# YunjiKim/Unsupervised-Keypoint-Learning-for-Guiding-Class-conditional-Video-Prediction

Measured on AMD Instinct MI355X. Metric: detector_translator train frames/sec @128x128 K=15, higher is better.
Workload: dtype f32

## Files before the change

include/kpx.h:

```cpp
#ifndef KPX_H
#define KPX_H

#include <stddef.h>
#include <stdint.h>

#ifdef __cplusplus
extern "C" {
#endif

#define KPX_EINVAL (-1)
#define KPX_ABI_VERSION 25

enum { KPX_ACT_NONE = 0, KPX_ACT_RELU = 1, KPX_ACT_LRELU = 2 , KPX_ACT_TANH = 3  };

int kpx_abi_version(void);

int kpx_reload_env(void);

enum { KPX_ARITH_F32 = 0, KPX_ARITH_BF16 = 1 };

size_t kpx_conv2d_fwd_workspace_bytes(int N, int Ho, int Wo, int Cin, int Cout, int KH, int KW);
int kpx_conv2d_fwd_f32(const float* x, int N, int Hi, int Wi, int Cin, int ldx,
                       const float* w_hwio, int KH, int KW, const float* bias,
                       float* y, int Ho, int Wo, int Cout, int ldy,
// ... 65 lines not shown
                         float* moving_mean, float* moving_var, float decay, float* y, int ldy, int act, void* scratch, void* stream);
int kpx_bn_train_bwd_f32(const float* dy, int lddy, const float* x, int ldx, size_t P, int groups, int C,
                         const float* mean, const float* invstd, const float* gamma, const float* beta, int act,
                         float* dx, int lddx, float* dgamma, float* dbeta, int accumulate,
                         const float* tile_stats, size_t tiles_per_group, void* scratch, void* stream);
int kpx_bn_train_fwd_bf16(const void* x, size_t P, int groups, int C, int ldx, const float* tile_stats, size_t tiles_per_group,
                          float eps, const float* gamma, const float* beta, float* mean, float* invstd,
                          float* moving_mean, float* moving_var, float decay, void* y, int ldy, int y_f32, int act, void* scratch, void* stream);
int kpx_bn_train_bwd_bf16(const void* dy, int lddy, int dy_f32, const void* x, int ldx, size_t P, int groups, int C,
                          const float* mean, const float* invstd, const float* gamma, const float* beta, int act,
                          void* dx, int lddx, float* dgamma, float* dbeta, int accumulate,
                          const float* tile_stats, size_t tiles_per_group, void* scratch, void* stream);
int kpx_bn_invstd_f32(const float* var, int C, float eps, float* invstd, void* stream);
int kpx_bn_apply_f32(const float* x, size_t P, int C, int ldx, const float* mean, const float* invstd,
                     const float* gamma, const float* beta, float* y, int ldy, int act, void* stream);
int kpx_bn_fold_conv_f32(const float* w, const float* bias, size_t rows, int C, const float* gamma, const float* beta,
                         const float* moving_mean, const float* moving_var, float eps, float* w_out, float* b_out, void* stream);

int kpx_conv3x3_wino43_eligible(int N, int H, int W, int K, int Nn, int ldin, const void* in_ptr);
size_t kpx_wino43_u_bytes(int Cin, int Cout);
int kpx_wino43_filter_transform_f32(const float* w_hwio, int Cin, int Cout, int dgrad, float* u, void* stream);
int kpx_wino43_filter_transform_batch_f32(const void* descs_dev, int n, void* stream);
int kpx_conv3x3_wino43_f32(const float* in, int N, int H, int W, int K, int ldin, const float* u, const float* bias,
                           float* out, int Nn, int ldout, int act, const float* mask_y, int ld_mask, float* pool_y, int ld_pool,
                           float* tile_stats, const float* bn_y, int ld_bn_y, const float* bn_beta, void* stream);
size_t kpx_conv3x3_wino43_stats_tiles(int N, int H, int W);
int kpx_conv3x3_wino43b_eligible(int N, int H, int W, int K, int Nn, int ldin, const void* in_ptr);
size_t kpx_wino43b_u_bytes(int Cin, int Cout);
int kpx_wino43b_filter_transform_f32(const float* w_hwio, int Cin, int Cout, int dgrad, void* u, void* stream);
int kpx_wino43b_filter_transform_batch_f32(const void* descs_dev, int n, void* stream);
int kpx_conv3x3_wino43b_f32(const float* in, int N, int H, int W, int K, int ldin, const void* u, const float* bias,
                            float* out, int Nn, int ldout, int act, const float* mask_y, int ld_mask, float* pool_y, int ld_pool,
                            float* tile_stats, const float* bn_y, int ld_bn_y, const float* bn_beta, void* stream);
int kpx_conv3x3_c16_eligible(int N, int H, int W, int K, int Nn, int ldin, int ldout, const void* in_ptr);
int kpx_conv3x3_c16_f32(const float* in, int N, int H, int W, int K, int ldin, const float* w_hwio, int dgrad, const float* bias,
                        float* out, int ldout, int act, float* tile_stats, void* stream);
int kpx_resize2x_fwd_f32(const float* x, int N, int H, int W, int C, int ldx, float* y, int ldy, void* stream);
int kpx_resize2x_bwd_f32(const float* dy, int N, int H, int W, int C, int lddy, float* dx, int lddx, void* stream);

int kpx_copy_channels_f32(const float* src, int ldsrc, float* dst, int lddst, size_t P, int C, void* stream);

size_t kpx_keypoint_head_scratch_bytes(int B, int H, int W, int K);
int kpx_keypoint_head_fwd_f32(const float* logits, int B, int H, int W, int K,
                              float* mu, float* prob_y, float* prob_x, void* scratch, void* stream);
int kpx_keypoint_head_bwd_f32(const float* dmu, const float* mu, const float* prob_y, const float* prob_x,
                              int B, int H, int W, int K, float* dlogits, void* stream);

size_t kpx_keypoint_head_proj_scratch_bytes(int B, int H, int W, int C, int K);
int kpx_keypoint_head_proj_eligible(int B, int H, int W, int C, int K);
int kpx_keypoint_head_proj_fwd_f32(const float* x, const float* wk, const float* bias, int B, int H, int W, int C, int K,
                                   float* mu, float* prob_y, float* prob_x, float* xs_y, float* xs_x, void* scratch, void* stream);
int kpx_keypoint_head_proj_bwd_f32(const float* dmu, const float* mu, const float* prob_y, const float* prob_x,
                                   const float* xs_y, const float* xs_x, const float* wk, int B, int H, int W, int C, int K,
                                   float* dx, float* dw, float* db, int accumulate, void* scratch, void* stream);

int kpx_gaussian_maps_fwd_f32(const float* mu, int B, int K, int H, int W, double inv_std, float* maps, int ldy, void* stream);
int kpx_gaussian_maps_bwd_f32(const float* dmaps, int lddy, const float* mu, int B, int K, int H, int W, double inv_std,
                              float* dmu, void* stream);

int kpx_point_maps_rgb_f32(const float* mu, int N, int K, int H, int W, double inv_std, const float* colors, float* out, void* stream);

int kpx_point_seq_strip_rgb_f32(const float* mu, int N, int T, int K, int H, int W, double inv_std, const float* colors, int recolour,
                                float* out, void* stream);

#define KPX_SUMMARY_SLICES 64
enum { KPX_PREMAP_IDENTITY = 0, KPX_PREMAP_X255 = 1, KPX_PREMAP_UNIT255 = 2, KPX_PREMAP_UNIT255_CLIP = 3 };
// ... 264 lines not shown
```

unsupervised-keypoint-learning-for-guiding-class-conditional-video-prediction_amd/_lib.py:

```python
import ctypes
import os
from ctypes import c_double, c_float, c_int, c_size_t, c_void_p

import torch

_HERE = os.path.dirname(os.path.abspath(__file__))
LIB_PATH = os.environ.get('KPX_LIB') or os.path.join(_HERE, 'libkpx_hip.so')


class KpxError(RuntimeError):
    pass


if not os.path.exists(LIB_PATH):
    raise ImportError(
        'libkpx_hip.so not found at %s -- build it first: python -c "import __graft_entry__ as g; g.build()" '
        '(or `make -C %s/csrc`). There is no CPU / PyTorch fallback for the hot path.' % (LIB_PATH, _HERE))

lib = ctypes.CDLL(LIB_PATH)

P = c_void_p
ABI_VERSION = 25
SIGNATURES = {
    'kpx_abi_version': (c_int, []),
    'kpx_reload_env': (c_int, []),
    'kpx_conv2d_fwd_workspace_bytes': (c_size_t, [c_int, c_int, c_int, c_int, c_int, c_int, c_int]),
    'kpx_conv2d_fwd_f32': (c_int, [P, c_int, c_int, c_int, c_int, c_int, P, c_int, c_int, P,
                                   P, c_int, c_int, c_int, c_int, c_int, c_int, c_int, c_int, c_int, P, c_size_t, P]),
    'kpx_conv2d_dgrad_workspace_bytes': (c_size_t, [c_int, c_int, c_int, c_int, c_int, c_int, c_int, c_int]),
    'kpx_conv2d_dgrad_f32': (c_int, [P, c_int, c_int, c_int, c_int, c_int, P, c_int, c_int,
                                     P, c_int, c_int, c_int, c_int, c_int, c_int, c_int, c_int, P, c_size_t, P]),
    'kpx_conv2d_dgrad_act_f32': (c_int, [P, c_int, c_int, c_int, c_int, c_int, P, c_int, c_int,
                                         P, c_int, c_int, c_int, c_int, c_int, c_int, c_int, c_int, P, c_int, c_int, P, c_size_t, P]),
    'kpx_conv2d_wgrad_workspace_bytes': (c_size_t, [c_int, c_int, c_int, c_int, c_int, c_int, c_int]),
    'kpx_conv2d_wgrad_f32': (c_int, [P, c_int, c_int, c_int, c_int, c_int, P, c_int, c_int, c_int, c_int,
                                     P, c_int, c_int, c_int, c_int, c_int, c_int, P, c_size_t, P]),
    'kpx_conv2d_wgrad_plan': (c_int, [P, c_int, c_int, c_int, c_int, c_int, P, c_int, c_int, c_int, c_int,
                                      c_int, c_int, c_int, c_int, c_int, c_int, P, P, P]),
    'kpx_wino_u_bytes': (c_size_t, [c_int, c_int]),
    'kpx_wino_filter_transform_f32': (c_int, [P, c_int, c_int, c_int, P, P]),
    'kpx_wino_filter_transform_batch_f32': (c_int, [P, c_int, P]),
    'kpx_conv3x3_wino_eligible': (c_int, [c_int, c_int, c_int, c_int, c_int, c_int, P]),
    'kpx_conv3x3_wino_f32': (c_int, [P, c_int, c_int, c_int, c_int, c_int, P, P, P, c_int, c_int, c_int, P, P, c_int, P, P]),
    'kpx_conv3x3_c16_eligible': (c_int, [c_int, c_int, c_int, c_int, c_int, c_int, c_int, P]),
    'kpx_conv3x3_c16_f32': (c_int, [P, c_int, c_int, c_int, c_int, c_int, P, c_int, P, P, c_int, c_int, P, P]),
    'kpx_conv3x3_wino43_eligible': (c_int, [c_int, c_int, c_int, c_int, c_int, c_int, P]),
    'kpx_wino43_u_bytes': (c_size_t, [c_int, c_int]),
    'kpx_wino43_filter_transform_f32': (c_int, [P, c_int, c_int, c_int, P, P]),
    'kpx_wino43_filter_transform_batch_f32': (c_int, [P, c_int, P]),
    'kpx_conv3x3_wino43_f32': (c_int, [P, c_int, c_int, c_int, c_int, c_int, P, P, P, c_int, c_int, c_int, P, c_int, P, c_int, P, P, c_int, P, P]),
    'kpx_conv3x3_wino43b_eligible': (c_int, [c_int, c_int, c_int, c_int, c_int, c_int, P]),
    'kpx_wino43b_u_bytes': (c_size_t, [c_int, c_int]),
    'kpx_wino43b_filter_transform_f32': (c_int, [P, c_int, c_int, c_int, P, P]),
    'kpx_wino43b_filter_transform_batch_f32': (c_int, [P, c_int, P]),
    'kpx_conv3x3_wino43b_f32': (c_int, [P, c_int, c_int, c_int, c_int, c_int, P, P, P, c_int, c_int, c_int, P, c_int, P, c_int, P, P, c_int, P, P]),
    'kpx_conv3x3_wino43_stats_tiles': (c_size_t, [c_int, c_int, c_int]),
    'kpx_conv3x3_wino_stats_tiles': (c_size_t, [c_int, c_int, c_int]),
    'kpx_conv3x3_bf16s_weights_bytes': (c_size_t, [c_int, c_int]),
    'kpx_conv3x3_bf16s_eligible': (c_int, [c_int, c_int, c_int, c_int, c_int, c_int, P]),
    'kpx_conv3x3_bf16s_stats_tiles': (c_int, [c_int, c_int, c_int, c_int, c_int]),
    'kpx_conv3x3_bf16s_prepare_f32': (c_int, [P, c_int, c_int, c_int, P, P]),
    'kpx_conv3x3_bf16s_prepare_batch_f32': (c_int, [P, c_int, P]),
    'kpx_conv3x3_bf16s': (c_int, [P, c_int, c_int, c_int, c_int, c_int, P, P, P, c_int, c_int, c_int, c_int, P, c_int, P, P]),
    'kpx_conv2d_fwd_bf16': (c_int, [P, c_int, c_int, c_int, c_int, c_int, P, c_int, c_int, P, P, c_int, c_int, c_int, c_int, c_int, c_int, c_int, c_int, c_int, P, c_size_t, P]),
    'kpx_conv2d_dgrad_bf16': (c_int, [P, c_int, c_int, c_int, c_int, c_int, P, c_int, c_int, P, c_int, c_int, c_int, c_int, c_int, c_int, c_int, c_int, P, c_int, c_int, P, c_size_t, P]),
    'kpx_conv2d_wgrad_bf16': (c_int, [P, c_int, c_int, c_int, c_int, c_int, P, c_int, c_int, c_int, c_int, P, c_int, c_int, c_int, c_int, c_int, P, c_size_t, P]),
    'kpx_conv_image_fwd_bf16': (c_int, [P, c_int, c_int, c_int, c_int, P, c_int, c_int, P, P, c_int, c_int, c_int, c_int, c_int, c_int, c_int, c_int, P]),
    'kpx_conv_image_dgrad_bf16': (c_int, [P, c_int, c_int, c_int, c_int, c_int, P, c_int, c_int, P, c_int, c_int, c_int, c_int, c_int, c_int, c_int, P]),
    'kpx_conv_image_wgrad_bf16': (c_int, [P, c_int, c_int, c_int, c_int, c_int, P, c_int, c_int, c_int, c_int, P, c_int, c_int, c_int, c_int, c_int, P, c_size_t, P]),
    'kpx_conv3x3_wgrad_bf16_eligible': (c_int, [c_int, c_int, c_int, c_int, c_int, c_int, c_int, P, P]),
    'kpx_conv3x3_wgrad_bf16_workspace_bytes': (c_size_t, [c_int, c_int, c_int, c_int, c_int]),
    'kpx_conv3x3_wgrad_bf16': (c_int, [P, c_int, c_int, c_int, c_int, c_int, P, c_int, c_int, P, P, c_size_t, P]),
    'kpx_conv3x3_bf16s_bnbwd': (c_int, [P, c_int, c_int, c_int, c_int, c_int, P, P, c_int, c_int, P, c_int, P, P, P]),
    'kpx_cast_channels': (c_int, [P, c_int, P, c_int, c_size_t, c_int, c_int, P]),
    'kpx_chan_sum_bf16': (c_int, [P, c_size_t, c_int, c_int, P, P, P]),
    'kpx_bn_train_fwd_bf16': (c_int, [P, c_size_t, c_int, c_int, c_int, P, c_size_t, c_float, P, P, P, P, P, P, c_float, P, c_int, c_int, c_int, P, P]),
    'kpx_bn_train_bwd_bf16': (c_int, [P, c_int, c_int, P, c_int, c_size_t, c_int, c_int, P, P, P, P, c_int, P, c_int, P, P, c_int, P, c_size_t, P, P]),
    'kpx_act_bwd_bf16': (c_int, [P, P, P, c_size_t, c_int, P]),
    'kpx_resize2x_fwd_bf16': (c_int, [P, c_int, c_int, c_int, c_int, c_int, P, c_int, P]),
    'kpx_resize2x_bwd_bf16': (c_int, [P, c_int, c_int, c_int, c_int, c_int, P, c_int, P]),
    'kpx_maxpool2_fwd_bf16': (c_int, [P, c_int, c_int, c_int, c_int, P, P]),
    'kpx_vgg_feat_bwd_bf16': (c_int, [P, c_size_t, P, c_float, P, c_int, c_int, c_int, c_int, P, P]),
    'kpx_l1_pair_fwd_bf16': (c_int, [P, c_size_t, P, P, P]),
    'kpx_act_bwd_f32': (c_int, [P, P, P, c_size_t, c_int, P]),
    'kpx_chan_reduce_scratch_bytes': (c_size_t, [c_int]),
    'kpx_chan_sum_f32': (c_int, [P, c_size_t, c_int, c_int, P, P, P]),
    'kpx_bn_invstd_f32': (c_int, [P, c_int, c_float, P, P]),
    'kpx_bn_fold_conv_f32': (c_int, [P, P, c_size_t, c_int, P, P, P, P, c_float, P, P, P]),
# ... 111 lines not shown
```

unsupervised-keypoint-learning-for-guiding-class-conditional-video-prediction_amd/csrc/conv_wino43b.hip:

```cpp
#include "kpx_bf16.h"
#include "kpx_env.h"
#include "wino43_options.h"
#include <type_traits>

#define W4B_ROWSLOTS 146
#define W4B_ROWSLOTS_PACK 154
#define W4B_NPIECES 44
#define W4B_RAW_BYTES (W4B_NPIECES * 1024)
#define W4B_ACC_OFF (2 * W4B_RAW_BYTES)
#define W4B_NLDS 4
#ifndef W4B_DMA_IN_T
#define W4B_DMA_IN_T 1
#endif
#ifndef W4B_U_AUX
#define W4B_U_AUX 0
#endif
#ifndef W4B_RING
#define W4B_RING 6
#endif
#if W4B_RING == 6
#define W4B_RING3 18
#else
#define W4B_RING3 27
#endif
#define W4B_STR2(x) #x
#define W4B_STR(x) W4B_STR2(x)
#define W4B_EPI_BYTES (36 * 32 * 32 * 4)
#define W4B_MAIN_BYTES (W4B_ACC_OFF + 4 * W4B_NLDS * 4096)

struct Wino43bGeom {
    const float* x; float* y; const void* U; const float* bias;
    int N, H, W, Cin, ldx, Cout, ldy, act;
    int Kp, Np;
    int tiles_y, tiles_x;
    const float* mask_y; int ld_mask;
    float* pool_y; int ld_pool;
    float* stats;
    const float* bn_beta;
};

__device__ __forceinline__ void w4b_split8(const float* __restrict__ v, u32x4* __restrict__ f) {
#if defined(W4B_EXP) && (W4B_EXP & 1)
#pragma unroll
    for (int m = 0; m < 4; ++m) { f[0][m] = kpx_bits(v[2 * m]); f[1][m] = kpx_bits(v[2 * m + 1]); f[2][m] = kpx_bits(v[m]); }
    return;
#endif
#pragma unroll
    for (int m = 0; m < 4; ++m) {
        unsigned p[3];
        kpx_split2<3>(v[2 * m], v[2 * m + 1], p);
        f[0][m] = p[0]; f[1][m] = p[1]; f[2][m] = p[2];
    }
}

struct KpxWino43bDesc { const float* w; unsigned* u; int cin, cout, dgrad, reserved; };

__constant__ double w4b_G[6][3] = {{0.25, 0.0, 0.0}, {-1.0 / 6.0, -1.0 / 6.0, -1.0 / 6.0}, {-1.0 / 6.0, 1.0 / 6.0, -1.0 / 6.0},
                                   {1.0 / 24.0, 1.0 / 12.0, 1.0 / 6.0}, {1.0 / 24.0, -1.0 / 12.0, 1.0 / 6.0}, {0.0, 0.0, 1.0}};

__device__ __forceinline__ void w4b_transform_filter(const float* __restrict__ w, int Cin, int Cout, bool dg, size_t idx, int Kp, int Np, unsigned* __restrict__ Ub) {
    const int K = dg ? Cout : Cin, Nn = dg ? Cin : Cout;
    const int KS = Kp >> 4, NB = Np >> 5, C8 = Kp >> 3;
    const int n = (int)(idx % (size_t)Np);
    const int c8 = (int)((idx / (size_t)Np) % (size_t)C8), i = (int)(idx / ((size_t)Np * C8));
    const double gi0 = w4b_G[i][0], gi1 = w4b_G[i][1], gi2 = w4b_G[i][2];
    float u[6][8];
    float g[9][8];
    const bool vec = dg && 8 * c8 + 8 <= K && n < Nn && (Cout & 3) == 0 && ((reinterpret_cast<uintptr_t>(w) & 15) == 0);
    if (vec) {
#pragma unroll
        for (int tp = 0; tp < 9; ++tp) {
            const f32x4* src = reinterpret_cast<const f32x4*>(w + ((size_t)(8 - tp) * Cin + n) * Cout + 8 * c8);
            const f32x4 a = src[0], b = src[1];
#pragma unroll
            for (int e = 0; e < 4; ++e) { g[tp][e] = a[e]; g[tp][4 + e] = b[e]; }
        }
    } else {
#pragma unroll
        for (int tp = 0; tp < 9; ++tp)
#pragma unroll
            for (int e = 0; e < 8; ++e) {
                const int c = 8 * c8 + e;
                g[tp][e] = !(c < K && n < Nn) ? 0.f : dg ? w[((size_t)(8 - tp) * Cin + n) * Cout + c] : w[((size_t)tp * Cin + c) * Cout + n];
            }
    }
// ... 606 lines not shown
```

unsupervised-keypoint-learning-for-guiding-class-conditional-video-prediction_amd/csrc/kpx_bf16.h:

```cpp
#pragma once
#include "kpx_common.h"

typedef __bf16 bf16x8 __attribute__((ext_vector_type(8)));
typedef unsigned int u32x4 __attribute__((ext_vector_type(4)));
typedef unsigned int u32x2 __attribute__((ext_vector_type(2)));
typedef __attribute__((address_space(3))) void* lds_ptr_t;

#define KPX_BUF_OOB 0x7ffffff0

template <int V> struct kpx_ic { static constexpr int value = V; };

static inline bool kpx_aligned16(const void* a, const void* b = nullptr, const void* c = nullptr) {
    return ((((uintptr_t)a) | ((uintptr_t)b) | ((uintptr_t)c)) & 15) == 0;
}

__device__ __forceinline__ unsigned kpx_bits(float v) { return __builtin_bit_cast(unsigned, v); }
__device__ __forceinline__ float kpx_float(unsigned v) { return __builtin_bit_cast(float, v); }
__device__ __forceinline__ unsigned kpx_pack_hi(unsigned a, unsigned b) { return __builtin_amdgcn_perm(b, a, 0x07060302u); }
__device__ __forceinline__ unsigned kpx_pack2(float a, float b) {
    typedef __bf16 bf16x2 __attribute__((ext_vector_type(2)));
    const bf16x2 p = {(__bf16)a, (__bf16)b};
    return __builtin_bit_cast(unsigned, p);
}
__device__ __forceinline__ float kpx_bf_lo(unsigned v) { return __builtin_bit_cast(float, v << 16); }
__device__ __forceinline__ float kpx_bf_hi(unsigned v) { return __builtin_bit_cast(float, v & 0xffff0000u); }

template <int TERMS>
__device__ __forceinline__ void kpx_split2(float a, float b, unsigned* p) {
    const unsigned ua = kpx_bits(a), ub = kpx_bits(b);
    p[0] = kpx_pack_hi(ua, ub);
    if (TERMS > 1) {
        const float ra = a - kpx_float(ua & 0xffff0000u), rb = b - kpx_float(ub & 0xffff0000u);
        const unsigned va = kpx_bits(ra), vb = kpx_bits(rb);
        p[1] = kpx_pack_hi(va, vb);
        if (TERMS > 2) {
            const float sa = ra - kpx_float(va & 0xffff0000u), sb = rb - kpx_float(vb & 0xffff0000u);
            p[2] = kpx_pack_hi(kpx_bits(sa), kpx_bits(sb));
        }
    }
}
```

unsupervised-keypoint-learning-for-guiding-class-conditional-video-prediction_amd/ops.py:

```python
import collections as _collections
import os as _os
import struct as _struct
import weakref as _weakref
from fractions import Fraction

import numpy as np
import torch

from . import _lib
from ._lib import lib, check
from ._args import OPTIONAL, _Scratch, _ptr, _stream, _workspace, check_out, check_tensors, scratch
from .tool_ops import *
from .tool_ops import seq_nearest, NEAREST_GROUP, NEAREST_MAX_QUERIES, NEAREST_MAX_WINDOWS
from .tool_ops import points_resample, points_speed, RESAMPLE_MODES, RESAMPLE_MAX_POINTS, RESAMPLE_MAX_RATE
from .tool_ops import set_neighbours, prdc, SET_MAX_K, SET_MAX_DIM, SET_MAX_QUERIES, SET_MAX_REFS

ACT_NONE, ACT_RELU, ACT_LRELU, ACT_TANH = 0, 1, 2, 3
BN_EPS = 1e-5
BN_DECAY = 0.999


def _require_gpu(t):
    if not t.is_cuda:
        raise _lib.KpxError('kpx ops run on MI355X only (got a %s tensor); there is no CPU fallback' % t.device)
# ... 202 lines not shown
        check(lib.kpx_conv3x3_bf16s_prepare_f32(w.data_ptr(), cin, cout, 1 if dgrad else 0, wf.data_ptr(), _stream()), 'kpx_conv3x3_bf16s_prepare_f32')
        return wf
    if ent[1] is not None:
        ent[1].ensure_fresh('bf16s')
    return ent[0]


def _bf16s_conv(inp, ld_in, k, w, bias, out, ld_out, nn, act, dgrad, want_stats=False, mask=None):
    n, h, wd = inp.shape[0], inp.shape[1], inp.shape[2]
    out_f32 = out.dtype == torch.float32
    k = _bf16s_gathered(inp, ld_in, k)
    if not k:
        return None
    g = 4 if out_f32 else 8
    if nn % g:
        nn = (nn + g - 1) // g * g
        if ld_out < nn:
            return None
    if ld_out % g or not lib.kpx_conv3x3_bf16s_eligible(n, h, wd, k, nn, ld_in, inp.data_ptr()):
        return None
    if out.data_ptr() % 16 or (mask is not None and (out_f32 or mask.dtype != BF16 or mask.data_ptr() % 16)):
        return None
    wf = _bf16s_prepared(w, dgrad)
    slab = None
    if want_stats:
        tiles = lib.kpx_conv3x3_bf16s_stats_tiles(n, h, wd, k, nn)
        slab = torch.empty(tiles * 2 * nn, dtype=torch.float32, device=inp.device)
    check(lib.kpx_conv3x3_bf16s(inp.data_ptr(), n, h, wd, k, ld_in, wf.data_ptr(), _ptr(bias), out.data_ptr(), nn, ld_out, 1 if out_f32 else 0, act,
                                _ptr(mask), mask.stride(2) if mask is not None else 0, _ptr(slab), _stream()), 'kpx_conv3x3_bf16s')
    conv_kernel_uses_bf16s[0] += 1
    return Launched((slab, Fraction(tiles, n)) if want_stats else None)


conv_kernel_uses ={'wino43': 0, 'wino43b': 0}

WINO43 = _os.environ.get('KPX_WINO43', '1') != '0'
DEBUG_FINITE = _os.environ.get('KPX_DEBUG_FINITE', '0') == '1'
WINO43_MIN_WORKGROUPS = 0
WINO43_NMIN = 33
WINO43B = _os.environ.get('KPX_WINO43B', '1') != '0'
WINO43B_MAX_CHANNELS = 512


def _kn(cin, cout, dgrad):
    return (cout, cin) if dgrad else (cin, cout)


def _wino43b_form_wanted(k, nn):
    return WINO43B and k >= 16 and k % 4 == 0 and nn >= WINO43_NMIN and max(k, nn) <= WINO43B_MAX_CHANNELS


def _wino43_wanted(k, nn, dgrad, f43_fwd=True):
    return bool(WINO43 and k >= 16 and nn >= WINO43_NMIN and (dgrad or f43_fwd))


_Form = _collections.namedtuple('_Form', 'nbytes transform transform_batch dtype wanted desc_last')
_FORMS = {
    'wino': _Form(lambda cin, cout, dgrad: lib.kpx_wino_u_bytes(cin, cout), 'kpx_wino_filter_transform_f32',
                  'kpx_wino_filter_transform_batch_f32', torch.float32, lambda k, nn, dgrad, f43_fwd: True, lambda nn: 0),
    'wino43': _Form(lambda cin, cout, dgrad: lib.kpx_wino43_u_bytes(cin, cout), 'kpx_wino43_filter_transform_f32',
                    'kpx_wino43_filter_transform_batch_f32', torch.float32, _wino43_wanted, lambda nn: 0),
    'wino43b': _Form(lambda cin, cout, dgrad: lib.kpx_wino43b_u_bytes(cin, cout), 'kpx_wino43b_filter_transform_f32',
                     'kpx_wino43b_filter_transform_batch_f32', torch.uint8,
                     lambda k, nn, dgrad, f43_fwd: _wino43_wanted(k, nn, dgrad, f43_fwd) and _wino43b_form_wanted(k, nn), lambda nn: 0),
    'bf16s': _Form(lambda cin, cout, dgrad: lib.kpx_conv3x3_bf16s_weights_bytes(*_kn(cin, cout, dgrad)), 'kpx_conv3x3_bf16s_prepare_f32',
                   'kpx_conv3x3_bf16s_prepare_batch_f32', torch.uint8, lambda k, nn, dgrad, f43_fwd: True, lambda nn: (nn + 127) // 128 * 4),
}
_WINO_FORMS = ('wino', 'wino43', 'wino43b')

_filter_forms = {}


def _cached_u(form, w, dgrad):
    key = (form, w.data_ptr(), 1 if dgrad else 0)
    ent = _filter_forms.get(key)
    if ent is None:
        return None
    if (ent[2] is not None and ent[2]() is None) or ent[3] != (int(w.shape[2]), int(w.shape[3])):
        _filter_forms.pop(key, None)
        return None
    return ent


class FilterBank:
    wino_needed_in_bf16 = False

    def __init__(self, named_filters, device, attrs=None):
        attrs = attrs or {}
        self.version = 0
        self.synced = {'wino': -1, 'bf16s': -1}
        self._wino_fresh_ev = None
        self.filters = [(n, w) for n, w in named_filters if w.dim() == 4 and w.shape[0] == 3 and w.shape[1] == 3]
        self.device = device
        self.f43_fwd = [attrs.get(n, {}).get('f43_fwd', True) for n, _ in self.filters]
        self.tables = {}
        if not self.filters or torch.device(device).type != 'cuda':
            self.filters = []
            return
        for form in _WINO_FORMS:
            self._build(form)

# ... 84 lines not shown
    if WINO43B and 'wino43b' in forms and lib.kpx_conv3x3_wino43b_eligible(n, h, wd, k, nn, ld_in, in_ptr):
        plan.append(('wino43b', bn))
    if f32:
        plan += [('wino43', bn)] + ([('wino43', False)] if bn else [])
    return plan


def _wino43_run(plan, forms, inp, ld_in, k, bias, out, ld_out, nn, act, want_stats=False, bn_src=None, mask=None, pool=None):
    n, h, wd = inp.shape[0], inp.shape[1], inp.shape[2]
    for form, bn in plan:
        entry = 'kpx_conv3x3_wino43b_f32' if form == 'wino43b' else 'kpx_conv3x3_wino43_f32'
        tiles = lib.kpx_conv3x3_wino43_stats_tiles(n, h, wd)
        slab = torch.empty(tiles * 2 * nn, dtype=torch.float32, device=inp.device) if (want_stats or bn) else None
        rc = getattr(lib, entry)(inp.data_ptr(), n, h, wd, k, ld_in, forms[form][0].data_ptr(), None if bn else _ptr(bias), out.data_ptr(), nn,
                                 ld_out, ACT_NONE if bn else act, _ptr(mask), mask.shape[3] if mask is not None else 0, _ptr(pool),
                                 pool.shape[3] if pool is not None else 0, _ptr(slab), bn_src[0].data_ptr() if bn else None,
                                 bn_src[0].shape[3] if bn else 0, bn_src[1].data_ptr() if bn else None, _stream())
        if _took(rc, entry):
            conv_kernel_uses['wino43'] += 1
            if form == 'wino43b':
                conv_kernel_uses['wino43b'] += 1
            return Launched((slab, Fraction(tiles, n)) if slab is not None else None)
    return None


def _f43_forms(w, dgrad):
    return {form: ent for form in ('wino43', 'wino43b') if (ent := _cached_u(form, w, dgrad)) is not None}


def _wino_pretransformed(inp, ld_in, k, w, bias, out, ld_out, nn, act, dgrad, want_stats=False, bn_src=None, mask=None, pool_out=None):
    n, h, wd = inp.shape[0], inp.shape[1], inp.shape[2]
    vgg = mask is not None or pool_out is not None
    ent = _cached_u('wino', w, dgrad)
    if not vgg and (ent is None or not lib.kpx_conv3x3_wino_eligible(n, h, wd, k, nn, ld_in, inp.data_ptr())):
        return None
    forms = _f43_forms(w, dgrad)
    plan = _wino43_plan(n, h, wd, k, nn, ld_in, inp.data_ptr(), dgrad, forms, want_stats=want_stats, bn_src=bn_src is not None, vgg=vgg)
    if vgg and not plan:
        return None
    bank = (forms['wino43'] if vgg else ent)[1]
    if bank is not None:
        bank.ensure_fresh('wino')
    r = _wino43_run(plan, forms, inp, ld_in, k, bias, out, ld_out, nn, act, want_stats=want_stats, bn_src=bn_src, mask=mask, pool=pool_out)
    if r is not None or vgg:
        return r
    bn = bn_src is not None and dgrad and h % 16 == 0 and wd % 16 == 0
    stats = bn or (want_stats and h % 16 == 0 and wd % 16 == 0)
    tiles = lib.kpx_conv3x3_wino_stats_tiles(n, h, wd)
    slab = torch.empty(tiles * 2 * nn, dtype=torch.float32, device=inp.device) if stats else None
    check(lib.kpx_conv3x3_wino_f32(inp.data_ptr(), n, h, wd, k, ld_in, ent[0].data_ptr(), None if bn else _ptr(bias), out.data_ptr(), nn, ld_out,
                                   ACT_NONE if bn else act, _ptr(slab), bn_src[0].data_ptr() if bn else None, bn_src[0].shape[3] if bn else 0,
                                   bn_src[1].data_ptr() if bn else None, _stream()), 'kpx_conv3x3_wino_f32')
    return Launched((slab, Fraction(tiles, n)) if stats else None)


def conv3x3_same(inp, ld_in, k, w, bias, out, ld_out, nn, act, dgrad, *, want_stats=False, bn_src=None, mask=None, pool_out=None):
    if act == ACT_TANH:
        return None
    n, h, wd = inp.shape[0], inp.shape[1], inp.shape[2]
    if inp.dtype == BF16:
        if pool_out is not None:
            return None
        if dgrad and bn_src is not None and mask is None and out.dtype == BF16:
            r = _bf16s_bnbwd(inp, ld_in, k, w, out, ld_out, nn, bn_src[0], bn_src[1])
            if r is not None:
                return r
        return _bf16s_conv(inp, ld_in, k, w, bias, out, ld_out, nn, act, dgrad, want_stats=want_stats, mask=mask)
    if out.dtype != torch.float32:
        return None
    if mask is not None or pool_out is not None:
        return _wino_pretransformed(inp, ld_in, k, w, bias, out, ld_out, nn, act, dgrad, mask=mask, pool_out=pool_out)
    if nn == 16 and not (dgrad and bn_src is not None) and lib.kpx_conv3x3_c16_eligible(n, h, wd, k, nn, ld_in, ld_out, inp.data_ptr()):
        tiles = (h // 16) * (wd // 16)
        slab = torch.empty(n * tiles * 2 * 16, dtype=torch.float32, device=inp.device) if want_stats else None
        check(lib.kpx_conv3x3_c16_f32(inp.data_ptr(), n, h, wd, k, ld_in, w.data_ptr(), 1 if dgrad else 0, _ptr(bias), out.data_ptr(), ld_out, act,
                                      _ptr(slab), _stream()), 'kpx_conv3x3_c16_f32')
        return Launched((slab, Fraction(tiles)) if want_stats else None)
    if not dgrad and nn <= 4 and k <= 128 and n * h * wd >= 65536:
        return None
    return _wino_pretransformed(inp, ld_in, k, w, bias, out, ld_out, nn, act, dgrad, want_stats=want_stats, bn_src=bn_src)


def _is_3x3_same(kh, kw, stride, pad_t, pad_l, hi, wi, ho, wo):
    return kh == 3 and kw == 3 and stride == 1 and pad_t == 1 and pad_l == 1 and ho == hi and wo == wi

# ... 1118 lines not shown
```

Before: 1408.

## Add Winograd F(2,3) bf16-split MFMA conv kernel for mid-size 3x3 layers

Adds a new Winograd F(2x2,3x3) conv kernel that runs the element-wise products on bf16x3-split MFMA 32x32x16. It has its own filter-transform layout, double-buffered LDS input staging via buffer-load-to-LDS, and fused bias, activation, BN statistics and BN-backward epilogues. Layers with K>=64 that the F(4,3) path does not take are routed to it, provided the grid has enough workgroups. This replaces the older f32 Winograd kernel on those layers, and it costs an extra cached filter form plus new host-side dispatch logic.

```diff
diff --git a/include/kpx.h b/include/kpx.h
--- a/include/kpx.h
+++ b/include/kpx.h
@@ -121,6 +121,13 @@
 int kpx_conv3x3_wino43b_f32(const float* in, int N, int H, int W, int K, int ldin, const void* u, const float* bias,
                             float* out, int Nn, int ldout, int act, const float* mask_y, int ld_mask, float* pool_y, int ld_pool,
                             float* tile_stats, const float* bn_y, int ld_bn_y, const float* bn_beta, void* stream);
+int kpx_conv3x3_wino23b_eligible(int N, int H, int W, int K, int Nn, int ldin, const void* in_ptr);
+size_t kpx_wino23b_u_bytes(int Cin, int Cout);
+int kpx_wino23b_filter_transform_f32(const float* w_hwio, int Cin, int Cout, int dgrad, void* u, void* stream);
+int kpx_wino23b_filter_transform_batch_f32(const void* descs_dev, int n, void* stream);
+int kpx_conv3x3_wino23b_f32(const float* in, int N, int H, int W, int K, int ldin, const void* u, const float* bias,
+                            float* out, int Nn, int ldout, int act, float* tile_stats, const float* bn_y, int ld_bn_y,
+                            const float* bn_beta, void* stream);
 int kpx_conv3x3_c16_eligible(int N, int H, int W, int K, int Nn, int ldin, int ldout, const void* in_ptr);
 int kpx_conv3x3_c16_f32(const float* in, int N, int H, int W, int K, int ldin, const float* w_hwio, int dgrad, const float* bias,
                         float* out, int ldout, int act, float* tile_stats, void* stream);
diff --git a/unsupervised-keypoint-learning-for-guiding-class-conditional-video-prediction_amd/_lib.py b/unsupervised-keypoint-learning-for-guiding-class-conditional-video-prediction_amd/_lib.py
--- a/unsupervised-keypoint-learning-for-guiding-class-conditional-video-prediction_amd/_lib.py
+++ b/unsupervised-keypoint-learning-for-guiding-class-conditional-video-prediction_amd/_lib.py
@@ -54,6 +54,11 @@
     'kpx_wino43b_filter_transform_f32': (c_int, [P, c_int, c_int, c_int, P, P]),
     'kpx_wino43b_filter_transform_batch_f32': (c_int, [P, c_int, P]),
     'kpx_conv3x3_wino43b_f32': (c_int, [P, c_int, c_int, c_int, c_int, c_int, P, P, P, c_int, c_int, c_int, P, c_int, P, c_int, P, P, c_int, P, P]),
+    'kpx_conv3x3_wino23b_eligible': (c_int, [c_int, c_int, c_int, c_int, c_int, c_int, P]),
+    'kpx_wino23b_u_bytes': (c_size_t, [c_int, c_int]),
+    'kpx_wino23b_filter_transform_f32': (c_int, [P, c_int, c_int, c_int, P, P]),
+    'kpx_wino23b_filter_transform_batch_f32': (c_int, [P, c_int, P]),
+    'kpx_conv3x3_wino23b_f32': (c_int, [P, c_int, c_int, c_int, c_int, c_int, P, P, P, c_int, c_int, c_int, P, P, c_int, P, P]),
     'kpx_conv3x3_wino43_stats_tiles': (c_size_t, [c_int, c_int, c_int]),
     'kpx_conv3x3_wino_stats_tiles': (c_size_t, [c_int, c_int, c_int]),
     'kpx_conv3x3_bf16s_weights_bytes': (c_size_t, [c_int, c_int]),
diff --git a/unsupervised-keypoint-learning-for-guiding-class-conditional-video-prediction_amd/csrc/conv_wino23b.hip b/unsupervised-keypoint-learning-for-guiding-class-conditional-video-prediction_amd/csrc/conv_wino23b.hip
--- /dev/null
+++ b/unsupervised-keypoint-learning-for-guiding-class-conditional-video-prediction_amd/csrc/conv_wino23b.hip
@@ -0,0 +1,376 @@
+#include "kpx_bf16.h"
+#include "kpx_env.h"
+#include <type_traits>
+
+#define W2B_RS 84
+#define W2B_PIECES 6
+#define W2B_RAW_BYTES (4 * W2B_PIECES * 1024)
+#define W2B_EPI_BYTES (16 * 64 * 32 * 4)
+#define W2B_LDS_BYTES (W2B_EPI_BYTES + 4 * 8 * 8 * 4)
+#define W2B_STR2(x) #x
+#define W2B_STR(x) W2B_STR2(x)
+#define W2B_UNITS3 24
+
+struct Wino23bGeom {
+    const float* x; float* y; const void* U; const float* bias;
+    int N, H, W, Cin, ldx, Cout, ldy, act;
+    int Kp, Np;
+    int tiles_y, tiles_x;
+    float* stats;
+    const float* mask_y; int ld_mask;
+    const float* bn_beta;
+};
+
+struct KpxWino23bDesc { const float* w; unsigned* u; int cin, cout, dgrad, reserved; };
+
+__device__ __forceinline__ void w2b_transform_filter(const float* __restrict__ w, int Cin, int Cout, bool dg, size_t idx, int Kp, int Np, unsigned* __restrict__ Ub) {
+    const int K = dg ? Cout : Cin, Nn = dg ? Cin : Cout;
+    const int KS = Kp >> 4, NB = Np >> 5, C8 = Kp >> 3;
+    const int n = (int)(idx % (size_t)Np);
+    const int c8 = (int)((idx / (size_t)Np) % (size_t)C8), i = (int)(idx / ((size_t)Np * C8));
+    float g[9][8];
+    const bool vec = dg && 8 * c8 + 8 <= K && n < Nn && (Cout & 3) == 0 && ((reinterpret_cast<uintptr_t>(w) & 15) == 0);
+    if (vec) {
+#pragma unroll
+        for (int tp = 0; tp < 9; ++tp) {
+            const f32x4* src = reinterpret_cast<const f32x4*>(w + ((size_t)(8 - tp) * Cin + n) * Cout + 8 * c8);
+            const f32x4 a = src[0], b = src[1];
+#pragma unroll
+            for (int e = 0; e < 4; ++e) { g[tp][e] = a[e]; g[tp][4 + e] = b[e]; }
+        }
+    } else {
+#pragma unroll
+        for (int tp = 0; tp < 9; ++tp)
+#pragma unroll
+            for (int e = 0; e < 8; ++e) {
+                const int c = 8 * c8 + e;
+                g[tp][e] = !(c < K && n < Nn) ? 0.f : dg ? w[((size_t)(8 - tp) * Cin + n) * Cout + c] : w[((size_t)tp * Cin + c) * Cout + n];
+            }
+    }
+    float u[4][8];
+#pragma unroll
+    for (int e = 0; e < 8; ++e) {
+        float t[3];
+#pragma unroll
+        for (int q = 0; q < 3; ++q)
+            t[q] = i == 0 ? g[q][e] : i == 1 ? 0.5f * (g[q][e] + g[3 + q][e] + g[6 + q][e]) : i == 2 ? 0.5f * (g[q][e] - g[3 + q][e] + g[6 + q][e]) : g[6 + q][e];
+        u[0][e] = t[0];
+        u[1][e] = 0.5f * (t[0] + t[1] + t[2]);
+        u[2][e] = 0.5f * (t[0] - t[1] + t[2]);
+        u[3][e] = t[2];
+    }
+    const int ks = c8 >> 1, h = c8 & 1, nb = n >> 5, r = n & 31;
+#pragma unroll
+    for (int j = 0; j < 4; ++j) {
+        u32x4 f[3];
+        kpx_split8(u[j], f);
+        u32x4* const o = reinterpret_cast<u32x4*>(Ub + (((size_t)(4 * i + j) * KS + ks) * NB + nb) * 768) + (r + 32 * h);
+        o[0] = f[0]; o[64] = f[1]; o[128] = f[2];
+    }
+}
+__global__ __launch_bounds__(256) void wino23b_filter_transform_batch_kernel(const KpxWino23bDesc* __restrict__ descs) {
+    const KpxWino23bDesc d = descs[blockIdx.y];
+    const bool dg = d.dgrad != 0;
+    const int K = dg ? d.cout : d.cin, Nn = dg ? d.cin : d.cout;
+    const int Kp = (K + 15) & ~15, Np = (Nn + 63) & ~63;
+    const size_t total = (size_t)4 * (Kp / 8) * Np;
+    for (size_t idx = (size_t)blockIdx.x * 256 + threadIdx.x; idx < total; idx += (size_t)gridDim.x * 256)
+        w2b_transform_filter(d.w, d.cin, d.cout, dg, idx, Kp, Np, d.u);
+}
+__global__ __launch_bounds__(256) void wino23b_filter_transform_kernel(const float* __restrict__ w, int Cin, int Cout, int dgrad, int Kp, int Np, unsigned* __restrict__ Ub) {
+    const size_t total = (size_t)4 * (Kp / 8) * Np;
+    for (size_t idx = (size_t)blockIdx.x * 256 + threadIdx.x; idx < total; idx += (size_t)gridDim.x * 256)
+        w2b_transform_filter(w, Cin, Cout, dgrad != 0, idx, Kp, Np, Ub);
+}
+
+template <int RH, int CH>
+__device__ __forceinline__ void w2b_bt_d_b(const f32x4 (&e)[3][3], f32x4 (&o)[4]) {
+    f32x4 r[2][3];
+#pragma unroll
+    for (int b = 0; b < 3; ++b) {
+        if (RH == 0) { r[0][b] = e[0][b] - e[2][b]; r[1][b] = e[1][b] + e[2][b]; }
+        else { r[0][b] = e[1][b] - e[0][b]; r[1][b] = e[0][b] - e[2][b]; }
+    }
+#pragma unroll
+    for (int lr = 0; lr < 2; ++lr) {
+        if (CH == 0) { o[2 * lr] = r[lr][0] - r[lr][2]; o[2 * lr + 1] = r[lr][1] + r[lr][2]; }
+        else { o[2 * lr] = r[lr][1] - r[lr][0]; o[2 * lr + 1] = r[lr][0] - r[lr][2]; }
+    }
+}
+
+template <int RH, int CH>
+__device__ __forceinline__ void w2b_transform(const unsigned char* __restrict__ base, float (&v)[4][8]) {
+#pragma unroll
+    for (int j = 0; j < 2; ++j) {
+        f32x4 e[3][3];
+#pragma unroll
+        for (int a = 0; a < 3; ++a)
+#pragma unroll
+            for (int b = 0; b < 3; ++b) {
+                constexpr int coff[4] = {0, 4, 9, 13};
+                e[a][b] = *reinterpret_cast<const f32x4*>(base + ((RH + a) * W2B_RS + coff[CH + b] + j) * 16);
+            }
+        f32x4 o[4];
+        w2b_bt_d_b<RH, CH>(e, o);
+#pragma unroll
+        for (int lp = 0; lp < 4; ++lp)
+#pragma unroll
+            for (int q = 0; q < 4; ++q) v[lp][4 * j + q] = o[lp][q];
+    }
+}
+
+template <int STATS>
+__global__ __launch_bounds__(256, 1) void conv_wino23b_kernel(const Wino23bGeom g) {
+    extern __shared__ __attribute__((aligned(16))) unsigned char smem[];
+    const int t = threadIdx.x, lane = t & 63, wave = __builtin_amdgcn_readfirstlane(t >> 6);
+    int L = kpx_xcd_remap(blockIdx.x, gridDim.x);
+    const int ntc = g.Np / 64;
+    const int nti = L % ntc; L /= ntc;
+    const int bx = L % g.tiles_x; L /= g.tiles_x;
+    const int by = L % g.tiles_y;
+    const int n = L / g.tiles_y;
+    const int oy0 = by * 16, ox0 = bx * 16, n0 = nti * 64;
+    const int rh = wave >> 1, ch = wave & 1;
+    const int li = lane & 31, lh = lane >> 5;
+    const int KS = g.Kp >> 4, NB = g.Np >> 5;
+
+    f32x16 acc[4][2][2];
+#pragma unroll
+    for (int a = 0; a < 4; ++a)
+#pragma unroll
+        for (int b = 0; b < 2; ++b)
+#pragma unroll
+            for (int c = 0; c < 2; ++c)
+#pragma unroll
+                for (int r = 0; r < 16; ++r) acc[a][b][c][r] = 0.f;
+
+    const unsigned img_bytes = (unsigned)g.H * g.W * g.ldx * 4u;
+    const __amdgpu_buffer_rsrc_t rsx = __builtin_amdgcn_make_buffer_rsrc(const_cast<float*>(g.x) + (size_t)n * g.H * g.W * g.ldx, 0, img_bytes, 0x00020000);
+    unsigned dtail = 0;
+    int dv[W2B_PIECES];
+#pragma unroll
+    for (int i = 0; i < W2B_PIECES; ++i) {
+        const int S = (wave * W2B_PIECES + i) * 64 + lane;
+        const int row = S / W2B_RS, rs = S - row * W2B_RS;
+        const int pair = rs / 9, r9 = rs - pair * 9;
+        const int col = 2 * pair + (r9 >> 2), q = r9 & 3;
+        const int iy = oy0 - 1 + row, ix = ox0 - 1 + col;
+        const bool ok = r9 < 8 && pair < 9 && row < 18 && (unsigned)iy < (unsigned)g.H && (unsigned)ix < (unsigned)g.W;
+        dv[i] = ok ? ((iy * g.W + ix) * g.ldx + q * 4) * 4 : KPX_BUF_OOB;
+        if ((KS - 1) * 16 + q * 4 < g.Cin) dtail |= 1u << i;
+    }
+    auto dma = [&](int s, int buf) {
+        unsigned char* const dst = smem + buf * W2B_RAW_BYTES + wave * (W2B_PIECES * 1024);
+#pragma unroll
+        for (int i = 0; i < W2B_PIECES; ++i) {
+            const int vo = (s == KS - 1 && !((dtail >> i) & 1u)) ? KPX_BUF_OOB : dv[i];
+            __builtin_amdgcn_raw_ptr_buffer_load_lds(rsx, (lds_ptr_t)(dst + i * 1024), 16, vo, s * 64, 0, 0);
+        }
+    };
+    const __amdgpu_buffer_rsrc_t rsu = __builtin_amdgcn_make_buffer_rsrc(const_cast<void*>(g.U), 0, 16u * (unsigned)(KS * NB) * 3072u, 0x00020000);
+    const int ustep = NB * 3072;
+    int ubase[4];
+#pragma unroll
+    for (int lp = 0; lp < 4; ++lp)
+        ubase[lp] = __builtin_amdgcn_readfirstlane(((4 * (2 * rh + (lp >> 1)) + 2 * ch + (lp & 1)) * KS * NB + 2 * nti) * 3072);
+    u32x4 ub[4][2][3];
+
+    const int rbase = ((2 * (li >> 3)) * W2B_RS + 9 * (li & 7) + 2 * lh) * 16;
+
+    dma(0, 0);
+#pragma unroll
+    for (int lp = 0; lp < 4; ++lp)
+#pragma unroll
+        for (int nb = 0; nb < 2; ++nb)
+#pragma unroll
+            for (int tm = 0; tm < 3; ++tm)
+                ub[lp][nb][tm] = __builtin_bit_cast(u32x4, __builtin_amdgcn_raw_buffer_load_b128(rsu, lane * 16, ubase[lp] + nb * 3072 + tm * 1024, 0));
+    asm volatile("s_waitcnt vmcnt(" W2B_STR(W2B_UNITS3) ")" ::: "memory");
+    __builtin_amdgcn_s_barrier();
+
+    for (int it = 0; it < KS; ++it) {
+        const int buf = it & 1;
+        const bool more = it + 1 < KS;
+        if (more) dma(it + 1, buf ^ 1);
+        const int uvo = more ? lane * 16 : KPX_BUF_OOB;
+        const int unext = (it + 1) * ustep;
+#pragma unroll
+        for (int th = 0; th < 2; ++th) {
+            float v[4][8];
+            const unsigned char* const tb = smem + buf * W2B_RAW_BYTES + th * (8 * W2B_RS * 16) + rbase;
+            if (rh == 0) { if (ch == 0) w2b_transform<0, 0>(tb, v); else w2b_transform<0, 1>(tb, v); }
+            else { if (ch == 0) w2b_transform<1, 0>(tb, v); else w2b_transform<1, 1>(tb, v); }
+            u32x4 af[4][3];
+#pragma unroll
+            for (int lp = 0; lp < 4; ++lp) kpx_split8(v[lp], af[lp]);
+            constexpr int PA[6] = {1, 0, 2, 0, 1, 0}, PB[6] = {1, 2, 0, 1, 0, 0};
+#pragma unroll
+            for (int lp = 0; lp < 4; ++lp)
+#pragma unroll
+                for (int nb = 0; nb < 2; ++nb) {
+#pragma unroll
+                    for (int pr = 0; pr < 6; ++pr)
+                        acc[lp][th][nb] = __builtin_amdgcn_mfma_f32_32x32x16_bf16(__builtin_bit_cast(bf16x8, af[lp][PA[pr]]),
+                                                                                  __builtin_bit_cast(bf16x8, ub[lp][nb][PB[pr]]), acc[lp][th][nb], 0, 0, 0);
+                    if (th == 1) {
+#pragma unroll
+                        for (int tm = 0; tm < 3; ++tm)
+                            ub[lp][nb][tm] = __builtin_bit_cast(u32x4, __builtin_amdgcn_raw_buffer_load_b128(rsu, uvo, ubase[lp] + nb * 3072 + unext + tm * 1024, 0));
+                    }
+                }
+        }
+        if (more) {
+            asm volatile("s_waitcnt vmcnt(" W2B_STR(W2B_UNITS3) ")" ::: "memory");
+            __builtin_amdgcn_s_barrier();
+        }
+    }
+
+    float* const P = reinterpret_cast<float*>(smem);
+    float* const S = reinterpret_cast<float*>(smem + W2B_EPI_BYTES);
+    const int cq = t & 7;
+    const bool vec_ok = (g.ldy & 3) == 0 && ((reinterpret_cast<uintptr_t>(g.y) & 15) == 0);
+    const bool mask_vec = STATS == 2 && (g.ld_mask & 3) == 0 && ((reinterpret_cast<uintptr_t>(g.mask_y) & 15) == 0);
+#pragma unroll
+    for (int nb = 0; nb < 2; ++nb) {
+        __syncthreads();
+#pragma unroll
+        for (int lp = 0; lp < 4; ++lp) {
+            const int p = 4 * (2 * rh + (lp >> 1)) + 2 * ch + (lp & 1);
+#pragma unroll
+            for (int th = 0; th < 2; ++th)
+#pragma unroll
+                for (int r = 0; r < 16; ++r)
+                    P[((p * 64 + th * 32 + (r & 3) + 8 * (r >> 2) + 4 * lh) * 32) + li] = acc[lp][th][nb][r];
+        }
+        __syncthreads();
+        const int c0 = n0 + 32 * nb + cq * 4;
+        f32x4 bv = {0.f, 0.f, 0.f, 0.f}, bvec = {0.f, 0.f, 0.f, 0.f};
+        if (g.bias) {
+#pragma unroll
+            for (int e = 0; e < 4; ++e) if (c0 + e < g.Cout) bv[e] = g.bias[c0 + e];
+        }
+        if (STATS == 2) {
+#pragma unroll
+            for (int e = 0; e < 4; ++e) if (c0 + e < g.Cout) bvec[e] = g.bn_beta[c0 + e];
+        }
+        f32x4 st_s = {0.f, 0.f, 0.f, 0.f}, st_q = {0.f, 0.f, 0.f, 0.f};
+#pragma unroll
+        for (int it = 0; it < 2; ++it) {
+            const int tile = (t >> 3) + 32 * it;
+            f32x4 m[4][4];
+#pragma unroll
+            for (int a = 0; a < 4; ++a)
+#pragma unroll
+                for (int b = 0; b < 4; ++b) m[a][b] = *reinterpret_cast<const f32x4*>(&P[((a * 4 + b) * 64 + tile) * 32 + cq * 4]);
+            f32x4 pv[4][2];
+#pragma unroll
+            for (int a = 0; a < 4; ++a) { pv[a][0] = m[a][0] + m[a][1] + m[a][2]; pv[a][1] = m[a][1] - m[a][2] - m[a][3]; }
+            const int oy = oy0 + 2 * (tile >> 3), ox = ox0 + 2 * (tile & 7);
+#pragma unroll
+            for (int dy = 0; dy < 2; ++dy)
+#pragma unroll
+                for (int dx = 0; dx < 2; ++dx) {
+                    f32x4 v = (dy == 0 ? pv[0][dx] + pv[1][dx] + pv[2][dx] : pv[1][dx] - pv[2][dx] - pv[3][dx]) + bv;
+                    if (g.act == KPX_ACT_RELU) {
+#pragma unroll
+                        for (int e = 0; e < 4; ++e) v[e] = fmaxf(v[e], 0.f);
+                    } else if (g.act == KPX_ACT_LRELU) {
+#pragma unroll
+                        for (int e = 0; e < 4; ++e) v[e] = v[e] > 0.f ? v[e] : 0.01f * v[e];
+                    }
+                    if (oy + dy >= g.H || ox + dx >= g.W) continue;
+                    const size_t pix = (size_t)(n * g.H + oy + dy) * g.W + ox + dx;
+                    if (STATS == 2) {
+                        const float* my = g.mask_y + pix * g.ld_mask + c0;
+                        f32x4 yv = {0.f, 0.f, 0.f, 0.f};
+                        if (mask_vec && c0 + 3 < g.Cout) yv = *reinterpret_cast<const f32x4*>(my);
+                        else {
+#pragma unroll
+                            for (int e = 0; e < 4; ++e) if (c0 + e < g.Cout) yv[e] = my[e];
+                        }
+#pragma unroll
+                        for (int e = 0; e < 4; ++e) {
+                            const float dz = yv[e] > 0.f ? v[e] : 0.f;
+                            st_s[e] += dz; st_q[e] += dz * (yv[e] - bvec[e]);
+                        }
+                    } else if (STATS == 1) { st_s += v; st_q += v * v; }
+                    float* o = g.y + pix * g.ldy + c0;
+                    if (vec_ok && c0 + 3 < g.Cout) *reinterpret_cast<f32x4*>(o) = v;
+                    else {
+#pragma unroll
+                        for (int e = 0; e < 4; ++e) if (c0 + e < g.Cout) o[e] = v[e];
+                    }
+                }
+        }
+        if (STATS != 0) {
+#pragma unroll
+            for (int sh = 8; sh <= 32; sh <<= 1)
+#pragma unroll
+                for (int e = 0; e < 4; ++e) { st_s[e] += __shfl_xor(st_s[e], sh); st_q[e] += __shfl_xor(st_q[e], sh); }
+            if (lane < 8) {
+                *reinterpret_cast<f32x4*>(&S[(wave * 8 + lane) * 8]) = st_s;
+                *reinterpret_cast<f32x4*>(&S[(wave * 8 + lane) * 8 + 4]) = st_q;
+            }
+            __syncthreads();
+            if (t < 64) {
+                const int stat = t >> 5, c = t & 31;
+                const int si = (c >> 2) * 8 + stat * 4 + (c & 3);
+                const float r = ((S[si] + S[64 + si]) + S[128 + si]) + S[192 + si];
+                const size_t tile_id = ((size_t)n * g.tiles_y + by) * g.tiles_x + bx;
+                if (n0 + 32 * nb + c < g.Cout) g.stats[(tile_id * 2 + stat) * g.Cout + n0 + 32 * nb + c] = r;
+            }
+        }
+    }
+}
+
+static std::atomic<unsigned long long> w2b_attr_mask{0};
+
+extern "C" int kpx_conv3x3_wino23b_eligible(int N, int H, int W, int K, int Nn, int ldin, const void* in_ptr) {
+    if (kpx_env()->no_wino || N <= 0 || H <= 0 || W <= 0) return 0;
+    return K >= 64 && K % 4 == 0 && Nn >= 64 && ldin >= K && ldin % 4 == 0 && (((uintptr_t)in_ptr) & 15) == 0 &&
+           (size_t)H * W * ldin * 4 < 0x7fffff00u && (size_t)16 * ((K + 15) & ~15) * ((Nn + 63) & ~63) * 6 < 0x7fffff00u &&
+           (size_t)N * ((H + 15) / 16) * ((W + 15) / 16) * ((Nn + 63) / 64) < 0x7fffffffu;
+}
+extern "C" size_t kpx_wino23b_u_bytes(int Cin, int Cout) {
+    const size_t a = (size_t)((Cin + 15) & ~15) * ((Cout + 63) & ~63), b = (size_t)((Cout + 15) & ~15) * ((Cin + 63) & ~63);
+    return 16 * 6 * (a > b ? a : b);
+}
+extern "C" int kpx_wino23b_filter_transform_f32(const float* w_hwio, int Cin, int Cout, int dgrad, void* U, void* stream) {
+    if (!w_hwio || !U || Cin <= 0 || Cout <= 0) return KPX_EINVAL;
+    const int K = dgrad ? Cout : Cin, Nn = dgrad ? Cin : Cout;
+    const int Kp = (K + 15) & ~15, Np = (Nn + 63) & ~63;
+    size_t nb = ((size_t)4 * (Kp / 8) * Np + 255) / 256; if (nb > 2048) nb = 2048;
+    hipLaunchKernelGGL(wino23b_filter_transform_kernel, dim3((unsigned)nb), dim3(256), 0, kpx_stream(stream), w_hwio, Cin, Cout, dgrad, Kp, Np, (unsigned*)U);
+    return kpx_launch_status();
+}
+extern "C" int kpx_wino23b_filter_transform_batch_f32(const void* descs_dev, int n, void* stream) {
+    if (!descs_dev || n <= 0 || n > 65535) return KPX_EINVAL;
+    hipLaunchKernelGGL(wino23b_filter_transform_batch_kernel, dim3(64, (unsigned)n), dim3(256), 0, kpx_stream(stream), (const KpxWino23bDesc*)descs_dev);
+    return kpx_launch_status();
+}
+
+extern "C" int kpx_conv3x3_wino23b_f32(const float* in, int N, int H, int W, int K, int ldin, const void* U, const float* bias,
+                                       float* out, int Nn, int ldout, int act, float* tile_stats, const float* bn_y, int ld_bn_y,
+                                       const float* bn_beta, void* stream) {
+    if (!in || !U || !out || ldout < Nn || act < 0 || act > 2 || !kpx_conv3x3_wino23b_eligible(N, H, W, K, Nn, ldin, in)) return KPX_EINVAL;
+    if (tile_stats && (H % 16 || W % 16)) return KPX_EINVAL;
+    if ((bn_y || bn_beta) && (!tile_stats || !bn_y || !bn_beta || ld_bn_y < Nn || bias || act != KPX_ACT_NONE)) return KPX_EINVAL;
+    if (kpx_first_use_on_device(&w2b_attr_mask)) {
+        hipError_t e = hipFuncSetAttribute(reinterpret_cast<const void*>(conv_wino23b_kernel<0>), hipFuncAttributeMaxDynamicSharedMemorySize, W2B_LDS_BYTES);
+        if (e == hipSuccess) e = hipFuncSetAttribute(reinterpret_cast<const void*>(conv_wino23b_kernel<1>), hipFuncAttributeMaxDynamicSharedMemorySize, W2B_LDS_BYTES);
+        if (e == hipSuccess) e = hipFuncSetAttribute(reinterpret_cast<const void*>(conv_wino23b_kernel<2>), hipFuncAttributeMaxDynamicSharedMemorySize, W2B_LDS_BYTES);
+        if (e != hipSuccess) return -(int)e;
+    }
+    Wino23bGeom g{};
+    g.x = in; g.y = out; g.U = U; g.bias = bias; g.stats = tile_stats;
+    g.mask_y = bn_y; g.ld_mask = ld_bn_y; g.bn_beta = bn_beta;
+    g.N = N; g.H = H; g.W = W; g.Cin = K; g.ldx = ldin; g.Cout = Nn; g.ldy = ldout; g.act = act;
+    g.Kp = (K + 15) & ~15; g.Np = (Nn + 63) & ~63;
+    g.tiles_y = (H + 15) / 16; g.tiles_x = (W + 15) / 16;
+    const unsigned blocks = (unsigned)((size_t)N * g.tiles_y * g.tiles_x * (g.Np / 64));
+    hipStream_t s = kpx_stream(stream);
+    if (bn_y) hipLaunchKernelGGL((conv_wino23b_kernel<2>), dim3(blocks), dim3(256), W2B_LDS_BYTES, s, g);
+    else if (tile_stats) hipLaunchKernelGGL((conv_wino23b_kernel<1>), dim3(blocks), dim3(256), W2B_LDS_BYTES, s, g);
+    else hipLaunchKernelGGL((conv_wino23b_kernel<0>), dim3(blocks), dim3(256), W2B_LDS_BYTES, s, g);
+    return kpx_launch_status();
+}
diff --git a/unsupervised-keypoint-learning-for-guiding-class-conditional-video-prediction_amd/csrc/conv_wino43b.hip b/unsupervised-keypoint-learning-for-guiding-class-conditional-video-prediction_amd/csrc/conv_wino43b.hip
--- a/unsupervised-keypoint-learning-for-guiding-class-conditional-video-prediction_amd/csrc/conv_wino43b.hip
+++ b/unsupervised-keypoint-learning-for-guiding-class-conditional-video-prediction_amd/csrc/conv_wino43b.hip
@@ -45,12 +45,7 @@
     for (int m = 0; m < 4; ++m) { f[0][m] = kpx_bits(v[2 * m]); f[1][m] = kpx_bits(v[2 * m + 1]); f[2][m] = kpx_bits(v[m]); }
     return;
 #endif
-#pragma unroll
-    for (int m = 0; m < 4; ++m) {
-        unsigned p[3];
-        kpx_split2<3>(v[2 * m], v[2 * m + 1], p);
-        f[0][m] = p[0]; f[1][m] = p[1]; f[2][m] = p[2];
-    }
+    kpx_split8(v, f);
 }
 
 struct KpxWino43bDesc { const float* w; unsigned* u; int cin, cout, dgrad, reserved; };
diff --git a/unsupervised-keypoint-learning-for-guiding-class-conditional-video-prediction_amd/csrc/kpx_bf16.h b/unsupervised-keypoint-learning-for-guiding-class-conditional-video-prediction_amd/csrc/kpx_bf16.h
--- a/unsupervised-keypoint-learning-for-guiding-class-conditional-video-prediction_amd/csrc/kpx_bf16.h
+++ b/unsupervised-keypoint-learning-for-guiding-class-conditional-video-prediction_amd/csrc/kpx_bf16.h
@@ -39,3 +39,12 @@
         }
     }
 }
+
+__device__ __forceinline__ void kpx_split8(const float* __restrict__ v, u32x4* __restrict__ f) {
+#pragma unroll
+    for (int m = 0; m < 4; ++m) {
+        unsigned p[3];
+        kpx_split2<3>(v[2 * m], v[2 * m + 1], p);
+        f[0][m] = p[0]; f[1][m] = p[1]; f[2][m] = p[2];
+    }
+}
diff --git a/unsupervised-keypoint-learning-for-guiding-class-conditional-video-prediction_amd/ops.py b/unsupervised-keypoint-learning-for-guiding-class-conditional-video-prediction_amd/ops.py
--- a/unsupervised-keypoint-learning-for-guiding-class-conditional-video-prediction_amd/ops.py
+++ b/unsupervised-keypoint-learning-for-guiding-class-conditional-video-prediction_amd/ops.py
@@ -258,7 +258,7 @@
     return Launched((slab, Fraction(tiles, n)) if want_stats else None)
 
 
-conv_kernel_uses ={'wino43': 0, 'wino43b': 0}
+conv_kernel_uses = {'wino43': 0, 'wino43b': 0, 'wino23b': 0}
 
 WINO43 = _os.environ.get('KPX_WINO43', '1') != '0'
 DEBUG_FINITE = _os.environ.get('KPX_DEBUG_FINITE', '0') == '1'
@@ -278,6 +278,25 @@
 
 def _wino43_wanted(k, nn, dgrad, f43_fwd=True):
     return bool(WINO43 and k >= 16 and nn >= WINO43_NMIN and (dgrad or f43_fwd))
+
+
+WINO23B = _os.environ.get('KPX_WINO23B', '1') != '0'
+WINO23B_MIN_WORKGROUPS = 256
+
+
+def _wino23b_wanted(k, nn, dgrad, f43_fwd=True):
+    return bool(WINO23B and k >= 64 and k % 4 == 0 and nn >= 64 and not _wino43_wanted(k, nn, dgrad, f43_fwd))
+
+
+def _wino23b_takes(n, h, wd, k, nn, ld_in, in_ptr):
+    if not WINO23B:
+        return False
+    if h % 16 == 0 and wd % 16 == 0:
+        if n * (h // 16) * (wd // 16) * ((nn + 63) // 64) < WINO23B_MIN_WORKGROUPS:
+            return False
+    elif not (h > 16 and wd > 16):
+        return False
+    return bool(lib.kpx_conv3x3_wino23b_eligible(n, h, wd, k, nn, ld_in, in_ptr))
 
 
 _Form = _collections.namedtuple('_Form', 'nbytes transform transform_batch dtype wanted desc_last')
@@ -289,10 +308,12 @@
     'wino43b': _Form(lambda cin, cout, dgrad: lib.kpx_wino43b_u_bytes(cin, cout), 'kpx_wino43b_filter_transform_f32',
                      'kpx_wino43b_filter_transform_batch_f32', torch.uint8,
                      lambda k, nn, dgrad, f43_fwd: _wino43_wanted(k, nn, dgrad, f43_fwd) and _wino43b_form_wanted(k, nn), lambda nn: 0),
+    'wino23b': _Form(lambda cin, cout, dgrad: lib.kpx_wino23b_u_bytes(cin, cout), 'kpx_wino23b_filter_transform_f32',
+                     'kpx_wino23b_filter_transform_batch_f32', torch.uint8, _wino23b_wanted, lambda nn: 0),
     'bf16s': _Form(lambda cin, cout, dgrad: lib.kpx_conv3x3_bf16s_weights_bytes(*_kn(cin, cout, dgrad)), 'kpx_conv3x3_bf16s_prepare_f32',
                    'kpx_conv3x3_bf16s_prepare_batch_f32', torch.uint8, lambda k, nn, dgrad, f43_fwd: True, lambda nn: (nn + 127) // 128 * 4),
 }
-_WINO_FORMS = ('wino', 'wino43', 'wino43b')
+_WINO_FORMS = ('wino', 'wino43', 'wino43b', 'wino23b')
 
 _filter_forms = {}
 
@@ -443,13 +464,16 @@
     n, h, wd = inp.shape[0], inp.shape[1], inp.shape[2]
     vgg = mask is not None or pool_out is not None
     ent = _cached_u('wino', w, dgrad)
-    if not vgg and (ent is None or not lib.kpx_conv3x3_wino_eligible(n, h, wd, k, nn, ld_in, inp.data_ptr())):
+    ent23 = None if vgg else _cached_u('wino23b', w, dgrad)
+    if ent23 is not None and not _wino23b_takes(n, h, wd, k, nn, ld_in, inp.data_ptr()):
+        ent23 = None
+    if not vgg and ent23 is None and (ent is None or not lib.kpx_conv3x3_wino_eligible(n, h, wd, k, nn, ld_in, inp.data_ptr())):
         return None
     forms = _f43_forms(w, dgrad)
     plan = _wino43_plan(n, h, wd, k, nn, ld_in, inp.data_ptr(), dgrad, forms, want_stats=want_stats, bn_src=bn_src is not None, vgg=vgg)
     if vgg and not plan:
         return None
-    bank = (forms['wino43'] if vgg else ent)[1]
+    bank = (forms['wino43'] if vgg else ent23 if ent23 is not None else ent)[1]
     if bank is not None:
         bank.ensure_fresh('wino')
     r = _wino43_run(plan, forms, inp, ld_in, k, bias, out, ld_out, nn, act, want_stats=want_stats, bn_src=bn_src, mask=mask, pool=pool_out)
@@ -459,9 +483,12 @@
     stats = bn or (want_stats and h % 16 == 0 and wd % 16 == 0)
     tiles = lib.kpx_conv3x3_wino_stats_tiles(n, h, wd)
     slab = torch.empty(tiles * 2 * nn, dtype=torch.float32, device=inp.device) if stats else None
-    check(lib.kpx_conv3x3_wino_f32(inp.data_ptr(), n, h, wd, k, ld_in, ent[0].data_ptr(), None if bn else _ptr(bias), out.data_ptr(), nn, ld_out,
-                                   ACT_NONE if bn else act, _ptr(slab), bn_src[0].data_ptr() if bn else None, bn_src[0].shape[3] if bn else 0,
-                                   bn_src[1].data_ptr() if bn else None, _stream()), 'kpx_conv3x3_wino_f32')
+    entry, u = ('kpx_conv3x3_wino23b_f32', ent23[0]) if ent23 is not None else ('kpx_conv3x3_wino_f32', ent[0])
+    check(getattr(lib, entry)(inp.data_ptr(), n, h, wd, k, ld_in, u.data_ptr(), None if bn else _ptr(bias), out.data_ptr(), nn, ld_out,
+                              ACT_NONE if bn else act, _ptr(slab), bn_src[0].data_ptr() if bn else None, bn_src[0].shape[3] if bn else 0,
+                              bn_src[1].data_ptr() if bn else None, _stream()), entry)
+    if ent23 is not None:
+        conv_kernel_uses['wino23b'] += 1
     return Launched((slab, Fraction(tiles, n)) if stats else None)
 
 
```

Result: no change. 1418, median of 6 (+0.7%).
